# qqueing/DeepSpeaker-pytorch

Hardware: AMD Instinct MI355X
Metric: embeddings/sec (64-fbank x 160-frame utterances) (higher is better)
Workload: dtype f16

## Files before the change

deepspeaker-pytorch_amd/csrc/conv_block_f16.hip:

```cpp
#include <ds_device.h>
#include <algorithm>
#include <type_traits>
#include "ds_common.h"
#include "conv_mfma_f16_parts.h"

namespace {

constexpr int BK_R = 8;
constexpr int BK_CK = 32;
constexpr int BK_PS = 80;

struct BlockK {
    const _Float16 *x;
    const _Float16 *wa, *wb;
    const float *sa, *ha, *sb, *hb;
    void *y;
    int B, H, W, C;
    int tiles_per_img, n_tiles;
    int flags;
    unsigned y_bytes, x_bytes, y_plane_stride;
    const int *lens;
    int xcd_slots;
    unsigned *sched;
    int sched_lds;
#ifdef DS_F16_PROBE
    long long *probe;
#endif
};

#ifdef DS_F16_PROBE
#define DS_BLK_STAMP(i) do { if (p.probe && threadIdx.x == 0 && tile_no < 4) p.probe[((size_t)blockIdx.x * 4 + tile_no) * 8 + (i)] = (long long)__builtin_amdgcn_s_memtime(); } while (0)
#else
#define DS_BLK_STAMP(i) ((void)0)
#endif

#ifndef DS_BLOCK_RING
#define DS_BLOCK_RING 6
#endif

template <int WM, int WN, int NIT, bool MASKED = false>
__global__ void __launch_bounds__(WM * WN * 64) DS_ONE_WAVE_PER_SIMD conv_block3x3_f16_kernel(const BlockK p) {
    constexpr int NTHR = WM * WN * 64;
    constexpr int W = 16 * WM, WSH = WM == 2 ? 5 : 4;
    constexpr int MSA = 5, MSB = 4, NSUB = 2;
    constexpr int NT = 9, NU = 2 * NT, RU = DS_BLOCK_RING;
    constexpr int NMFA = MSA * NSUB, NMFB = MSB * NSUB;
    constexpr int SPU = (NMFA + 1) / 2 - NSUB;
    constexpr int UL = (NIT + SPU - 1) / SPU;
    constexpr int SPUB = NMFB / 2 - NSUB;
    constexpr int ROWS_A = BK_R + 2, ROWS_IN = BK_R + 4;
    using EG = ds_f16_epi<NSUB>;
    constexpr int TP = EG::TP, LPP = EG::LPP, PPI = EG::PPI, NRI = EG::NRI;
    constexpr int NRES = MSB * NRI, ULR = (NRES + SPUB - 1) / SPUB;
    static_assert(WM == 1 || WM == 2, "map width 16 or 32");
    static_assert(2 * UL <= NU && ULR + 2 <= NU && NU % RU == 0, "not enough units for the staging traffic");
    static_assert(NIT * NTHR == ROWS_IN * W * 4, "staging items must tile the input rows exactly");
    constexpr unsigned OOB = 0x80000000u;
    constexpr int pitch = W + 2;
    constexpr int tileA_bytes = ROWS_IN * pitch * BK_PS;

    char *lds = (char *)ds_dynamic_lds();
    const int tid = threadIdx.x, lane = tid & 63, wave = tid >> 6;
    const int wm = wave / WN, wn = wave % WN;
    const int l31 = lane & 31, lhi = lane >> 5;
    constexpr int C = WM == 2 ? 64 : 128;
    constexpr int RSB = C * 2 + 16;
    constexpr int n_chunks = C / BK_CK;
    const int n_base = wn * NSUB * 32;
    size_t lane_w = ds_f16_lane_w(n_base, l31, lhi);
    const size_t w_kc_stride = (size_t)NT * C * 16, w_tap_stride = (size_t)C * 16;
    auto w_unit = [&](const _Float16 *w, int chunk, int u) {
        return ds_f16_w_unit<NT, BK_CK / 16>(w, lane_w, w_kc_stride, w_tap_stride, chunk, u);
    };

    const int xcd = (int)blockIdx.x & 7, slot0 = (int)blockIdx.x >> 3;
    const int my_imgs = p.xcd_slots > 0 ? (p.B - xcd + 7) / 8 : 0;
    int t_cur = p.xcd_slots > 0 ? slot0 : (int)blockIdx.x;
    const int t_static = p.xcd_slots > 0 ? p.xcd_slots : (int)gridDim.x;
    const int t_end = p.xcd_slots > 0 ? my_imgs * p.tiles_per_img : p.n_tiles;
    unsigned *const q_next = p.sched + (p.xcd_slots > 0 ? xcd : 0);
    int *const sched_word = (int *)(lds + p.sched_lds);
    if (tid == 0) *sched_word = t_static + (int)ds_atomic_inc(q_next);
    __syncthreads();
    int t_next = ds_uniform(*sched_word);
    const float rcp_tpi = 1.0f / (float)p.tiles_per_img;
    auto tile_of = [&](int t, int &b, int &r0) {
        const int im = ds_div_small(t, p.tiles_per_img, rcp_tpi);
        r0 = (t - im * p.tiles_per_img) * BK_R;
        b = p.xcd_slots > 0 ? im * 8 + xcd : im;
    };

    unsigned g_rel[NIT];
    int l_off[NIT];
    {
        const int q = tid & 3, pix0 = tid >> 2;
#pragma unroll
        for (int it = 0; it < NIT; ++it) {
            const int pix = pix0 + it * (NTHR / 4);
            const int vr = pix >> WSH, c = pix & (W - 1);
            g_rel[it] = (unsigned)((pix * C + q * 8) * 2);
            l_off[it] = (vr * pitch + c + 1) * BK_PS + q * 16;
        }
    }
    const int lpix = ds_mfma_lpix(l31);
    int a_off[MSA];
#pragma unroll
    for (int ms = 0; ms < MSA; ++ms) {
        const int m = (wm * MSA + ms) * 32 + lpix;
        a_off[ms] = ((m >> WSH) * pitch + (m & (W - 1))) * BK_PS + 16 * lhi;
    }
    auto tap_off = [&](int tt, int rs) { return ((tt / 3) * pitch + (tt % 3)) * rs; };
    const ds_buffer ybuf = ds_make_buffer(p.y, p.y_bytes);
    const ds_buffer rbuf = ds_make_buffer(p.x, p.x_bytes);
    const int x_row_bytes = W * C * 2;
    const int my_c = (lane % LPP) * 8, my_p = lane / LPP;
    const int col = n_base + my_c;
    const bool out32 = (p.flags & DS_EPI_OUT_F32) != 0;
    float *tb = (float *)lds + wave * (2 * 32 * TP);

    auto stage_window = [&](int b, int r0, ds_buffer &xb, unsigned &lo) {
        const int h0 = r0 - 2;
        const int first = h0 < 0 ? -h0 : 0;
        const int last = p.H - h0 < ROWS_IN ? p.H - h0 : ROWS_IN;
        lo = (unsigned)(first * x_row_bytes);
        xb = ds_make_buffer((const char *)p.x + (size_t)(b * p.H + h0 + first) * x_row_bytes,
                            (unsigned)((last > first ? last - first : 0) * x_row_bytes));
    };

    f16x8 bq[RU][NSUB];
#pragma unroll
    for (int d = 0; d < RU; ++d)
#pragma unroll
        for (int ns = 0; ns < NSUB; ++ns) bq[d][ns] = *(const f16x8 *)(w_unit(p.wa, 0, d) + (size_t)ns * 32 * 16);

    f32x16 acc[MSA][NSUB];
    const f32x16 zero16 = {0.f, 0.f, 0.f, 0.f, 0.f, 0.f, 0.f, 0.f, 0.f, 0.f, 0.f, 0.f, 0.f, 0.f, 0.f, 0.f};

    f32x4 st[NIT];
    int b = 0, r0 = 0;
    ds_buffer xbuf = rbuf;
    unsigned x_lo = 0;
    if (t_cur < t_end) {
        tile_of(t_cur, b, r0);
        stage_window(b, r0, xbuf, x_lo);
#pragma unroll
        for (int it = 0; it < NIT; ++it) st[it] = ds_buffer_load_f32x4(xbuf, g_rel[it] - x_lo);
    }

    int tile_no = 0;
    (void)tile_no;
    for (; t_cur < t_end; ++tile_no) {
        DS_BLK_STAMP(0);
        int t_drawn = 0;
        if (tid == 0) t_drawn = t_static + (int)ds_atomic_inc(q_next);
        DS_OPAQUE_VGPR(lane_w);
        int h_valid = p.H;
        if (MASKED) {
            const int len = p.lens[b];
            h_valid = len < p.H ? len : p.H;
        }
        ds_lds_barrier();
        for (int i = tid; i < 2 * ROWS_IN * 2 * (BK_PS / 16); i += NTHR) {
            const int piece = i % (BK_PS / 16), rec = i / (BK_PS / 16);
            const int side = rec & 1, row = (rec >> 1) % ROWS_IN, buf = (rec >> 1) / ROWS_IN;
            *(f32x4 *)(lds + buf * tileA_bytes + (row * pitch + side * (W + 1)) * BK_PS + 16 * piece) = f32x4{0.0f, 0.0f, 0.0f, 0.0f};
        }
#pragma unroll
        for (int it = 0; it < NIT; ++it) *(f32x4 *)(lds + l_off[it]) = st[it];
        ds_lds_barrier();
        DS_BLK_STAMP(1);

        auto run_chunk = [&](auto first_tag, auto last_tag, int chunk, const char *buf, char *obuf) __attribute__((always_inline)) {
            constexpr bool FIRST = decltype(first_tag)::value, LAST = decltype(last_tag)::value;
            f16x8 a[2][MSA];
#pragma unroll
            for (int ms = 0; ms < MSA; ++ms) {
                DS_OPAQUE_VGPR(a_off[ms]);
                a[0][ms] = *(const f16x8 *)(buf + a_off[ms] + tap_off(0, BK_PS));
            }
            const unsigned xn = (unsigned)((chunk + 1) * BK_CK * 2) - x_lo;
            __builtin_amdgcn_sched_barrier(0);
#pragma unroll
            for (int u = 0; u < NU; ++u) {
                const int cur = u & 1, slot = u % RU;
                const bool more = u + 1 < NU;
                const char *nfrag = buf + tap_off((u + 1) % NT, BK_PS) + 32 * ((u + 1) / NT);
                const int ur = u - 1 + RU;
                const _Float16 *rw = (LAST && ur >= NU) ? w_unit(p.wb, 0, ur - NU)
                                                        : w_unit(p.wa, ur >= NU ? chunk + 1 : chunk, ur >= NU ? ur - NU : ur);
                const int rslot = (u + RU - 1) % RU;
#pragma unroll
                for (int q = 0; q < NMFA; ++q) {
                    const int ms = q / NSUB, ns = q % NSUB;
                    acc[ms][ns] = ds_mfma_32x32x16_f16(bq[slot][ns], a[cur][ms], (FIRST && u == 0) ? zero16 : acc[ms][ns]);
                    if (q & 1) {
                        const int lm = q >> 1;
#ifndef DS_ABL_NO_AFRAG
                        if (lm < MSA && more) a[cur ^ 1][lm] = *(const f16x8 *)(nfrag + a_off[lm]);
#endif
                    } else {
                        const int e = q >> 1;
                        if (e < NSUB) {
#ifndef DS_ABL_NO_REFILL
                            bq[rslot][e] = *(const f16x8 *)(rw + (size_t)e * 32 * 16);
#endif
                        } else if constexpr (!LAST) {
#ifndef DS_ABL_NO_STAGE
                            const int s = e - NSUB;
                            if (u < UL) {
                                const int it = u * SPU + s;
                                if (it < NIT) st[it] = ds_buffer_load_f32x4(xbuf, g_rel[it] + xn);
                            } else if (u >= NU - UL) {
                                const int it = (u - (NU - UL)) * SPU + s;
                                if (it < NIT) *(f32x4 *)(obuf + l_off[it]) = st[it];
                            }
#endif
                        }
                    }
                    __builtin_amdgcn_sched_barrier(0);
                }
            }
        };
        run_chunk(std::true_type{}, std::false_type{}, 0, lds, lds + tileA_bytes);
        ds_lds_barrier();
        for (int i = 1; i + 1 < n_chunks; ++i) {
            char *b0 = lds + (i & 1) * tileA_bytes, *b1 = lds + ((i & 1) ^ 1) * tileA_bytes;
            run_chunk(std::false_type{}, std::false_type{}, i, b0, b1);
            ds_lds_barrier();
        }
        run_chunk(std::false_type{}, std::true_type{}, n_chunks - 1, lds + ((n_chunks - 1) & 1) * tileA_bytes, lds);
        DS_BLK_STAMP(2);

        {
            f32x4 sca[NSUB][4], sha[NSUB][4];
#pragma unroll
            for (int ns = 0; ns < NSUB; ++ns)
#pragma unroll
                for (int g = 0; g < 4; ++g) {
                    const int c0 = n_base + ns * 32 + 8 * g + 4 * lhi;
                    sca[ns][g] = *(const f32x4 *)(p.sa + c0);
                    sha[ns][g] = *(const f32x4 *)(p.ha + c0);
                }
            ds_lds_barrier();
            const int ppr = RSB / 16;
            for (int i = tid; i < ROWS_A * 2 * ppr; i += NTHR) {
                const int piece = i % ppr, rec = i / ppr;
                *(f32x4 *)(lds + ((rec >> 1) * pitch + (rec & 1) * (W + 1)) * RSB + 16 * piece) = f32x4{0.0f, 0.0f, 0.0f, 0.0f};
            }
#pragma unroll
            for (int ms = 0; ms < MSA; ++ms) {
                const int m = (wm * MSA + ms) * 32 + lpix;
                const int i = m >> WSH, c = m & (W - 1);
                const int row = r0 - 1 + i;
                const unsigned keep = (row >= 0 && row < h_valid) ? 0xFFFFFFFFu : 0u;
                char *rec = lds + (i * pitch + c + 1) * RSB;
#pragma unroll
                for (int ns = 0; ns < NSUB; ++ns)
#pragma unroll
                    for (int g = 0; g < 4; ++g) {
                        ds_u32x2 hb;
#pragma unroll
                        for (int j2 = 0; j2 < 2; ++j2) {
                            const ds_f32x2 v = {acc[ms][ns][4 * g + 2 * j2], acc[ms][ns][4 * g + 2 * j2 + 1]};
                            const ds_f32x2 sc2 = {sca[ns][g][2 * j2], sca[ns][g][2 * j2 + 1]};
                            const ds_f32x2 sh2 = {sha[ns][g][2 * j2], sha[ns][g][2 * j2 + 1]};
                            ds_f32x2 t = v * sc2 + sh2;
                            t[0] = fminf(fmaxf(t[0], DS_F16_CLIP_LO), DS_F16_CLIP_HI);
                            t[1] = fminf(fmaxf(t[1], DS_F16_CLIP_LO), DS_F16_CLIP_HI);
                            hb[j2] = __builtin_bit_cast(unsigned, __builtin_convertvector(t, ds_f16x2)) & keep;
                        }
                        *(ds_u32x2 *)(rec + (n_base + ns * 32 + 8 * g + 4 * lhi) * 2) = hb;
                    }
            }
            ds_lds_barrier();
        }
        DS_BLK_STAMP(3);

        const int lin_base = (b * p.H + r0) * W;
        const int lin_valid = (p.H - r0 < BK_R ? p.H - r0 : BK_R) * W;
        f32x4 resv[MSB][NRI];
        {
            const int total = n_chunks * NU;
            int b_off[MSB];
#pragma unroll
            for (int ms = 0; ms < MSB; ++ms) {
                const int m = (wm * MSB + ms) * 32 + lpix;
                b_off[ms] = ((m >> WSH) * pitch + (m & (W - 1))) * RSB + 16 * lhi;
            }
            f16x8 a[2][MSB];
#pragma unroll
            for (int ms = 0; ms < MSB; ++ms) {
                DS_OPAQUE_VGPR(b_off[ms]);
                a[0][ms] = *(const f16x8 *)(lds + b_off[ms] + tap_off(0, RSB));
            }
            __builtin_amdgcn_sched_barrier(0);
            auto run_b = [&](auto first_tag, auto last_tag, int chunk) __attribute__((always_inline)) {
                constexpr bool FIRSTB = decltype(first_tag)::value, LASTB = decltype(last_tag)::value;
#pragma unroll
                for (int u = 0; u < NU; ++u) {
                    const int cur = u & 1, slot = u % RU;
                    const int gu = chunk * NU + u;
                    const bool more = gu + 1 < total;
                    const int nu = (u + 1) % NU, nchunk = (u + 1 < NU) ? chunk : chunk + 1;
                    const char *nfrag = lds + tap_off(nu % NT, RSB) + 32 * (nu / NT) + (more ? nchunk : chunk) * 64;
                    const int ur = u - 1 + RU;
                    const int rchunk = ur >= NU ? chunk + 1 : chunk;
                    const _Float16 *rw = rchunk < n_chunks ? w_unit(p.wb, rchunk, ur >= NU ? ur - NU : ur)
                                                           : w_unit(p.wa, 0, ur >= NU ? ur - NU : ur);
                    const int rslot = (u + RU - 1) % RU;
#pragma unroll
                    for (int q = 0; q < NMFB; ++q) {
                        const int ms = q / NSUB, ns = q % NSUB;
                        acc[ms][ns] = ds_mfma_32x32x16_f16(bq[slot][ns], a[cur][ms], (FIRSTB && u == 0) ? zero16 : acc[ms][ns]);
                        if (q & 1) {
                            const int lm = q >> 1;
#ifndef DS_ABL_NO_AFRAG
                            if (lm < MSB) a[cur ^ 1][lm] = *(const f16x8 *)(nfrag + b_off[lm]);
#endif
                        } else {
                            const int e = q >> 1;
                            if (e < NSUB) {
#ifndef DS_ABL_NO_REFILL
                                bq[rslot][e] = *(const f16x8 *)(rw + (size_t)e * 32 * 16);
#endif
                            } else if constexpr (LASTB) {
                                const int ri = (u - (NU - 2 - ULR)) * SPUB + (e - NSUB);
                                if (u >= NU - 2 - ULR && ri < NRES) {
                                    const int rms = ri / NRI, rk = ri % NRI;
                                    const int m = (wm * MSB + rms) * 32 + rk * PPI + my_p;
#ifdef DS_ABL_NO_RES
                                    resv[rms][rk] = f32x4{0.f, 0.f, 0.f, 0.f};
#else
                                    resv[rms][rk] = ds_buffer_load_f32x4(rbuf, m < lin_valid ? (unsigned)((lin_base + m) * C + col) * 2u
                                                                                            : DS_BUFFER_OOB);
#endif
                                }
                            }
                        }
                        __builtin_amdgcn_sched_barrier(0);
                    }
                }
            };
            run_b(std::true_type{}, std::false_type{}, 0);
            for (int chunk = 1; chunk + 1 < n_chunks; ++chunk) run_b(std::false_type{}, std::false_type{}, chunk);
            run_b(std::false_type{}, std::true_type{}, n_chunks - 1);
        }

        DS_BLK_STAMP(4);
        if (tid == 0) *sched_word = t_drawn;
        ds_lds_barrier();
        DS_BLK_STAMP(5);
        const int t_after = ds_uniform(*sched_word);
#ifndef DS_EPI_TABLES_LATE
        const f32x4 sc[2] = {*(const f32x4 *)(p.sb + col), *(const f32x4 *)(p.sb + col + 4)};
        const f32x4 sh[2] = {*(const f32x4 *)(p.hb + col), *(const f32x4 *)(p.hb + col + 4)};
        __builtin_amdgcn_sched_barrier(0);
#endif
        int nb = b, nr0 = r0;
        {
            const bool has_next = t_next < t_end;
            if (has_next) {
                tile_of(t_next, nb, nr0);
                stage_window(nb, nr0, xbuf, x_lo);
            } else {
                xbuf = ds_make_buffer(p.x, 0u);
                x_lo = 0;
            }
#pragma unroll
            for (int it = 0; it < NIT; ++it) st[it] = ds_buffer_load_f32x4(xbuf, g_rel[it] - x_lo);
        }
        const int lin_kept = (h_valid - r0) * W;
#ifdef DS_EPI_TABLES_LATE
        __builtin_amdgcn_sched_barrier(0);
        const f32x4 sc[2] = {*(const f32x4 *)(p.sb + col), *(const f32x4 *)(p.sb + col + 4)};
        const f32x4 sh[2] = {*(const f32x4 *)(p.hb + col), *(const f32x4 *)(p.hb + col + 4)};
#endif
        auto put_tile = [&](int ms) { ds_f16_put_tile<NSUB>(tb + (ms & 1) * (32 * TP), acc[ms], lpix, lhi); };
        const unsigned y_mul = p.y_plane_stride ? 16u : (unsigned)C;
        const unsigned y_add = p.y_plane_stride ? (unsigned)(col >> 4) * p.y_plane_stride + (unsigned)(col & 15) : (unsigned)col;
        auto write_out = [&](auto f32_tag) __attribute__((always_inline)) {
            constexpr bool OUT32 = decltype(f32_tag)::value;
            put_tile(0);
#pragma unroll
            for (int ms = 0; ms < MSB; ++ms) {
                const int cb = ms & 1;
                ds_wave_sync();
                const float *src = tb + cb * (32 * TP);
                f32x4 tv[NRI][2];
#pragma unroll
                for (int k = 0; k < NRI; ++k)
#pragma unroll
                    for (int hq = 0; hq < 2; ++hq) tv[k][hq] = *(const f32x4 *)(src + (k * PPI + my_p) * TP + my_c + 4 * hq);
                if (ms + 1 < MSB) put_tile(ms + 1);
#pragma unroll
                for (int k = 0; k < NRI; ++k) {
                    const f16x8 r8 = __builtin_bit_cast(f16x8, resv[ms][k]);
                    const int m = (wm * MSB + ms) * 32 + k * PPI + my_p;
                    const float keep = (!MASKED || m < lin_kept) ? DS_F16_CLIP_HI : DS_F16_CLIP_LO;
                    f32x4 o[2];
#pragma unroll
                    for (int hq = 0; hq < 2; ++hq)
#pragma unroll
                        for (int j2 = 0; j2 < 2; ++j2) {
                            const ds_f32x2 v = {tv[k][hq][2 * j2], tv[k][hq][2 * j2 + 1]};
                            const ds_f32x2 s2 = {sc[hq][2 * j2], sc[hq][2 * j2 + 1]}, h2 = {sh[hq][2 * j2], sh[hq][2 * j2 + 1]};
                            const ds_f16x2 rh = {r8[4 * hq + 2 * j2], r8[4 * hq + 2 * j2 + 1]};
                            ds_f32x2 t = v * s2 + h2;
                            t = t + __builtin_convertvector(rh, ds_f32x2);
                            o[hq][2 * j2] = fminf(fmaxf(t[0], DS_F16_CLIP_LO), keep);
                            o[hq][2 * j2 + 1] = fminf(fmaxf(t[1], DS_F16_CLIP_LO), keep);
                        }
                    const unsigned vo = m < lin_valid ? (unsigned)(lin_base + m) * y_mul + y_add : DS_BUFFER_OOB;
                    if constexpr (OUT32) {
                        const unsigned bo = vo != DS_BUFFER_OOB ? vo * 4u : DS_BUFFER_OOB;
                        ds_buffer_store_out_f32x4(ybuf, bo, o[0]);
                        ds_buffer_store_out_f32x4(ybuf, bo != DS_BUFFER_OOB ? bo + 16u : DS_BUFFER_OOB, o[1]);
                    } else {
                        ds_u32x4 hb;
#pragma unroll
                        for (int hq = 0; hq < 2; ++hq)
#pragma unroll
                            for (int j2 = 0; j2 < 2; ++j2)
                                hb[2 * hq + j2] = __builtin_bit_cast(unsigned, __builtin_convertvector(
                                                                                   ds_f32x2{o[hq][2 * j2], o[hq][2 * j2 + 1]}, ds_f16x2));
#ifdef DS_ABL_NO_STORE
                        if (hb[0] == 0x12345678u)
#endif
                        ds_buffer_store_out_f32x4(ybuf, vo != DS_BUFFER_OOB ? vo * 2u : DS_BUFFER_OOB, __builtin_bit_cast(f32x4, hb));
                    }
                }
            }
        };
        if (out32) write_out(std::true_type{});
        else write_out(std::false_type{});
        DS_BLK_STAMP(6);
        b = nb;
        r0 = nr0;
        t_cur = t_next;
        t_next = t_after;
    }
    if (tid == 0 && ds_atomic_inc(p.sched + DS_SCHED_DONE) == gridDim.x - 1) {
        for (int i = 0; i <= DS_SCHED_DONE; ++i) p.sched[i] = 0u;
    }
}

static size_t block_lds_bytes(int W, int C, int waves) {
    const size_t tileA = (size_t)(BK_R + 4) * (W + 2) * BK_PS;
    const size_t interm = (size_t)(BK_R + 2) * (W + 2) * (C * 2 + 16);
    const size_t epi = (size_t)2 * waves * 32 * ds_f16_epi<2>::TP * 4;
    return std::max(std::max(2 * tileA, interm), epi) + 64;
}

}

#ifdef DS_F16_PROBE
static long long *g_blk_probe = nullptr;
extern "C" void ds_block_set_probe(long long *buf) { g_blk_probe = buf; }
#endif


extern "C" int ds_conv_block_f16_supported(int B, int H, int W, int C) {
    if (B <= 0 || H <= 0) return 0;
    if ((long long)B * H * W * C >= (1ll << 30)) return 0;
    return (W == 32 && C == 64) || (W == 16 && C == 128);
}

static int conv_block_f16(const void *x_f16, const void *wa_f16, const void *wb_f16, const float *scale_a,
                          const float *shift_a, const float *scale_b, const float *shift_b, void *y, const int *lens,
                          int B, int H, int W, int C, int flags, void *stream) {
    DS_REQUIRE(x_f16 && wa_f16 && wb_f16 && scale_a && shift_a && scale_b && shift_b && y, DS_ERR_NULL);
    DS_REQUIRE(ds_conv_block_f16_supported(B, H, W, C), DS_ERR_UNSUPPORTED);
    DS_REQUIRE(DS_ALIGNED16(x_f16) && DS_ALIGNED16(wa_f16) && DS_ALIGNED16(wb_f16) && DS_ALIGNED16(y) &&
                   DS_ALIGNED16(scale_a) && DS_ALIGNED16(shift_a) && DS_ALIGNED16(scale_b) && DS_ALIGNED16(shift_b),
               DS_ERR_ALIGNMENT);
    DS_REQUIRE(!((flags & DS_EPI_OUT_F32) && (flags & DS_EPI_OUT_PLANES16)), DS_ERR_UNSUPPORTED);
    BlockK k;
    k.x = (const _Float16 *)x_f16; k.wa = (const _Float16 *)wa_f16; k.wb = (const _Float16 *)wb_f16;
    k.sa = scale_a; k.ha = shift_a; k.sb = scale_b; k.hb = shift_b; k.y = y;
    k.B = B; k.H = H; k.W = W; k.C = C;
    k.tiles_per_img = ds_ceil_div(H, BK_R);
    k.n_tiles = B * k.tiles_per_img;
    k.flags = flags;
    const long long n = (long long)B * H * W * C;
    k.x_bytes = (unsigned)(n * 2);
    k.y_bytes = (unsigned)(n * ((flags & DS_EPI_OUT_F32) ? 4 : 2));
    k.y_plane_stride = (flags & DS_EPI_OUT_PLANES16) ? (unsigned)((long long)B * H * W * 16) : 0u;
    k.lens = lens;
#ifdef DS_F16_PROBE
    k.probe = g_blk_probe;
#endif
    const int resident = 2 * ds_cu_count();
    int grid = k.n_tiles < resident ? k.n_tiles : resident;
    k.xcd_slots = 0;
    if (B >= 8 && grid == resident && resident % 8 == 0) k.xcd_slots = resident / 8;
    k.sched = ds_sched_slot(stream);
    DS_REQUIRE(k.sched != nullptr, DS_ERR_NO_WORKSPACE);
    k.sched_lds = (int)block_lds_bytes(W, C, 2) - 16;
    if (C == 64) {
        if (lens) DS_LAUNCH_BIG_LDS((conv_block3x3_f16_kernel<2, 1, 12, true>), grid, 128, block_lds_bytes(W, C, 2), stream, k);
        else DS_LAUNCH_BIG_LDS((conv_block3x3_f16_kernel<2, 1, 12>), grid, 128, block_lds_bytes(W, C, 2), stream, k);
    } else {
        if (lens) DS_LAUNCH_BIG_LDS((conv_block3x3_f16_kernel<1, 2, 6, true>), grid, 128, block_lds_bytes(W, C, 2), stream, k);
        else DS_LAUNCH_BIG_LDS((conv_block3x3_f16_kernel<1, 2, 6>), grid, 128, block_lds_bytes(W, C, 2), stream, k);
    }
    return ds_last_launch_error();
}

extern "C" int ds_conv_block_f16(const void *x_f16, const void *wa_f16, const void *wb_f16, const float *scale_a,
                                 const float *shift_a, const float *scale_b, const float *shift_b, void *y, int B, int H,
                                 int W, int C, int flags, void *stream) {
    return conv_block_f16(x_f16, wa_f16, wb_f16, scale_a, shift_a, scale_b, shift_b, y, nullptr, B, H, W, C, flags, stream);
}

extern "C" int ds_conv_block_f16_masked(const void *x_f16, const void *wa_f16, const void *wb_f16, const float *scale_a,
                                        const float *shift_a, const float *scale_b, const float *shift_b, void *y,
                                        const int *lens, int B, int H, int W, int C, int flags, void *stream) {
    DS_REQUIRE(lens != nullptr, DS_ERR_NULL);
    return conv_block_f16(x_f16, wa_f16, wb_f16, scale_a, shift_a, scale_b, shift_b, y, lens, B, H, W, C, flags, stream);
}
```

Baseline: 397,000.

## Cache BN tables in LDS, template output type, rework tile scheduling draw

Copies the four batch-norm scale/shift vectors into LDS once per block and reads epilogue tables from there instead of global memory. Makes the f32 output mode a template parameter so the epilogue branch is resolved at compile time. Replaces the float-reciprocal tile division with a host-computed magic multiplier, moves the atomic tile draw to after the compute and publishes it through LDS, and adds dummy out-of-bounds stores plus opaque-register and schedule barriers and extra probe stamps. The changes raise LDS use per block and add new sync ordering for the scheduler word.

```diff
diff --git a/deepspeaker-pytorch_amd/csrc/conv_block_f16.hip b/deepspeaker-pytorch_amd/csrc/conv_block_f16.hip
--- a/deepspeaker-pytorch_amd/csrc/conv_block_f16.hip
+++ b/deepspeaker-pytorch_amd/csrc/conv_block_f16.hip
@@ -17,6 +17,7 @@
     void *y;
     int B, H, W, C;
     int tiles_per_img, n_tiles;
+    unsigned tpi_magic;
     int flags;
     unsigned y_bytes, x_bytes, y_plane_stride;
     const int *lens;
@@ -29,16 +30,26 @@
 };
 
 #ifdef DS_F16_PROBE
-#define DS_BLK_STAMP(i) do { if (p.probe && threadIdx.x == 0 && tile_no < 4) p.probe[((size_t)blockIdx.x * 4 + tile_no) * 8 + (i)] = (long long)__builtin_amdgcn_s_memtime(); } while (0)
+#define DS_BLK_STAMP(i) do { if (p.probe && threadIdx.x == 0 && tile_no < 4) p.probe[((size_t)blockIdx.x * 4 + tile_no) * 24 + (i)] = (long long)__builtin_amdgcn_s_memtime(); } while (0)
+#define DS_BLK_STAMP_IN(i) do { __builtin_amdgcn_sched_barrier(0); DS_BLK_STAMP(i); __builtin_amdgcn_sched_barrier(0); } while (0)
 #else
 #define DS_BLK_STAMP(i) ((void)0)
+#define DS_BLK_STAMP_IN(i) ((void)0)
 #endif
 
 #ifndef DS_BLOCK_RING
 #define DS_BLOCK_RING 6
 #endif
 
-template <int WM, int WN, int NIT, bool MASKED = false>
+__device__ __forceinline__ unsigned blk_draw(unsigned *q) {
+#if defined(__HIP_DEVICE_COMPILE__)
+    return __builtin_amdgcn_atomic_inc32(q, 0xFFFFFFFFu, __ATOMIC_RELAXED, "agent");
+#else
+    return ds_atomic_inc(q);
+#endif
+}
+
+template <int WM, int WN, int NIT, bool MASKED = false, bool OUT32 = false>
 __global__ void __launch_bounds__(WM * WN * 64) DS_ONE_WAVE_PER_SIMD conv_block3x3_f16_kernel(const BlockK p) {
     constexpr int NTHR = WM * WN * 64;
     constexpr int W = 16 * WM, WSH = WM == 2 ? 5 : 4;
@@ -81,11 +92,18 @@
     unsigned *const q_next = p.sched + (p.xcd_slots > 0 ? xcd : 0);
     int *const sched_word = (int *)(lds + p.sched_lds);
     if (tid == 0) *sched_word = t_static + (int)ds_atomic_inc(q_next);
+    float *const bn_tab = (float *)(lds + p.sched_lds + 16);
+    for (int i = tid; i < C; i += NTHR) {
+        bn_tab[i] = p.sa[i];
+        bn_tab[C + i] = p.ha[i];
+        bn_tab[2 * C + i] = p.sb[i];
+        bn_tab[3 * C + i] = p.hb[i];
+    }
     __syncthreads();
     int t_next = ds_uniform(*sched_word);
-    const float rcp_tpi = 1.0f / (float)p.tiles_per_img;
     auto tile_of = [&](int t, int &b, int &r0) {
-        const int im = ds_div_small(t, p.tiles_per_img, rcp_tpi);
+        int im = (int)(((unsigned long long)(unsigned)t * p.tpi_magic) >> 32);
+        im += ((im + 1) * p.tiles_per_img <= t) ? 1 : 0;
         r0 = (t - im * p.tiles_per_img) * BK_R;
         b = p.xcd_slots > 0 ? im * 8 + xcd : im;
     };
@@ -115,7 +133,6 @@
     const int x_row_bytes = W * C * 2;
     const int my_c = (lane % LPP) * 8, my_p = lane / LPP;
     const int col = n_base + my_c;
-    const bool out32 = (p.flags & DS_EPI_OUT_F32) != 0;
     float *tb = (float *)lds + wave * (2 * 32 * TP);
 
     auto stage_window = [&](int b, int r0, ds_buffer &xb, unsigned &lo) {
@@ -145,14 +162,15 @@
         stage_window(b, r0, xbuf, x_lo);
 #pragma unroll
         for (int it = 0; it < NIT; ++it) st[it] = ds_buffer_load_f32x4(xbuf, g_rel[it] - x_lo);
+#pragma unroll
+        for (int i = 0; i < NRES * (OUT32 ? 2 : 1); ++i)
+            ds_buffer_store_out_f32x4(ybuf, DS_BUFFER_OOB - 16u * (unsigned)i, f32x4{0.0f, 0.0f, 0.0f, 0.0f});
     }
 
     int tile_no = 0;
     (void)tile_no;
     for (; t_cur < t_end; ++tile_no) {
         DS_BLK_STAMP(0);
-        int t_drawn = 0;
-        if (tid == 0) t_drawn = t_static + (int)ds_atomic_inc(q_next);
         DS_OPAQUE_VGPR(lane_w);
         int h_valid = p.H;
         if (MASKED) {
@@ -160,6 +178,7 @@
             h_valid = len < p.H ? len : p.H;
         }
         ds_lds_barrier();
+        t_next = ds_uniform(*sched_word);
         for (int i = tid; i < 2 * ROWS_IN * 2 * (BK_PS / 16); i += NTHR) {
             const int piece = i % (BK_PS / 16), rec = i / (BK_PS / 16);
             const int side = rec & 1, row = (rec >> 1) % ROWS_IN, buf = (rec >> 1) / ROWS_IN;
@@ -238,8 +257,8 @@
 #pragma unroll
                 for (int g = 0; g < 4; ++g) {
                     const int c0 = n_base + ns * 32 + 8 * g + 4 * lhi;
-                    sca[ns][g] = *(const f32x4 *)(p.sa + c0);
-                    sha[ns][g] = *(const f32x4 *)(p.ha + c0);
+                    sca[ns][g] = *(const f32x4 *)(bn_tab + c0);
+                    sha[ns][g] = *(const f32x4 *)(bn_tab + C + c0);
                 }
             ds_lds_barrier();
             const int ppr = RSB / 16;
@@ -247,6 +266,7 @@
                 const int piece = i % ppr, rec = i / ppr;
                 *(f32x4 *)(lds + ((rec >> 1) * pitch + (rec & 1) * (W + 1)) * RSB + 16 * piece) = f32x4{0.0f, 0.0f, 0.0f, 0.0f};
             }
+            DS_BLK_STAMP_IN(12);
 #pragma unroll
             for (int ms = 0; ms < MSA; ++ms) {
                 const int m = (wm * MSA + ms) * 32 + lpix;
@@ -271,6 +291,7 @@
                         }
                         *(ds_u32x2 *)(rec + (n_base + ns * 32 + 8 * g + 4 * lhi) * 2) = hb;
                     }
+                DS_BLK_STAMP_IN(13 + ms);
             }
             ds_lds_barrier();
         }
@@ -347,15 +368,12 @@
         }
 
         DS_BLK_STAMP(4);
-        if (tid == 0) *sched_word = t_drawn;
+        unsigned drawn = 0;
+        if (tid == 0) drawn = blk_draw(q_next);
         ds_lds_barrier();
         DS_BLK_STAMP(5);
-        const int t_after = ds_uniform(*sched_word);
-#ifndef DS_EPI_TABLES_LATE
-        const f32x4 sc[2] = {*(const f32x4 *)(p.sb + col), *(const f32x4 *)(p.sb + col + 4)};
-        const f32x4 sh[2] = {*(const f32x4 *)(p.hb + col), *(const f32x4 *)(p.hb + col + 4)};
-        __builtin_amdgcn_sched_barrier(0);
-#endif
+        const f32x4 sc[2] = {*(const f32x4 *)(bn_tab + 2 * C + col), *(const f32x4 *)(bn_tab + 2 * C + col + 4)};
+        const f32x4 sh[2] = {*(const f32x4 *)(bn_tab + 3 * C + col), *(const f32x4 *)(bn_tab + 3 * C + col + 4)};
         int nb = b, nr0 = r0;
         {
             const bool has_next = t_next < t_end;
@@ -370,20 +388,18 @@
             for (int it = 0; it < NIT; ++it) st[it] = ds_buffer_load_f32x4(xbuf, g_rel[it] - x_lo);
         }
         const int lin_kept = (h_valid - r0) * W;
-#ifdef DS_EPI_TABLES_LATE
-        __builtin_amdgcn_sched_barrier(0);
-        const f32x4 sc[2] = {*(const f32x4 *)(p.sb + col), *(const f32x4 *)(p.sb + col + 4)};
-        const f32x4 sh[2] = {*(const f32x4 *)(p.hb + col), *(const f32x4 *)(p.hb + col + 4)};
-#endif
         auto put_tile = [&](int ms) { ds_f16_put_tile<NSUB>(tb + (ms & 1) * (32 * TP), acc[ms], lpix, lhi); };
         const unsigned y_mul = p.y_plane_stride ? 16u : (unsigned)C;
         const unsigned y_add = p.y_plane_stride ? (unsigned)(col >> 4) * p.y_plane_stride + (unsigned)(col & 15) : (unsigned)col;
-        auto write_out = [&](auto f32_tag) __attribute__((always_inline)) {
-            constexpr bool OUT32 = decltype(f32_tag)::value;
+        auto write_out = [&]() __attribute__((always_inline)) {
+            DS_BLK_STAMP_IN(7);
             put_tile(0);
 #pragma unroll
             for (int ms = 0; ms < MSB; ++ms) {
                 const int cb = ms & 1;
+                __builtin_amdgcn_sched_barrier(0);
+#pragma unroll
+                for (int k = 0; k < NRI; ++k) DS_OPAQUE_VGPR(resv[ms][k]);
                 ds_wave_sync();
                 const float *src = tb + cb * (32 * TP);
                 f32x4 tv[NRI][2];
@@ -429,27 +445,28 @@
                         ds_buffer_store_out_f32x4(ybuf, vo != DS_BUFFER_OOB ? vo * 2u : DS_BUFFER_OOB, __builtin_bit_cast(f32x4, hb));
                     }
                 }
+                DS_BLK_STAMP_IN(8 + ms);
             }
         };
-        if (out32) write_out(std::true_type{});
-        else write_out(std::false_type{});
+        write_out();
         DS_BLK_STAMP(6);
         b = nb;
         r0 = nr0;
+        if (tid == 0) *sched_word = t_static + (int)drawn;
         t_cur = t_next;
-        t_next = t_after;
     }
     if (tid == 0 && ds_atomic_inc(p.sched + DS_SCHED_DONE) == gridDim.x - 1) {
         for (int i = 0; i <= DS_SCHED_DONE; ++i) p.sched[i] = 0u;
     }
 }
 
-static size_t block_lds_bytes(int W, int C, int waves) {
+static size_t block_sched_lds(int W, int C, int waves) {
     const size_t tileA = (size_t)(BK_R + 4) * (W + 2) * BK_PS;
     const size_t interm = (size_t)(BK_R + 2) * (W + 2) * (C * 2 + 16);
     const size_t epi = (size_t)2 * waves * 32 * ds_f16_epi<2>::TP * 4;
-    return std::max(std::max(2 * tileA, interm), epi) + 64;
-}
+    return std::max(std::max(2 * tileA, interm), epi) + 64 - 16;
+}
+static size_t block_lds_bytes(int W, int C, int waves) { return block_sched_lds(W, C, waves) + 16 + (size_t)4 * C * sizeof(float); }
 
 }
 
@@ -480,6 +497,7 @@
     k.B = B; k.H = H; k.W = W; k.C = C;
     k.tiles_per_img = ds_ceil_div(H, BK_R);
     k.n_tiles = B * k.tiles_per_img;
+    k.tpi_magic = k.tiles_per_img == 1 ? 0xFFFFFFFFu : (unsigned)((1ull << 32) / (unsigned)k.tiles_per_img);
     k.flags = flags;
     const long long n = (long long)B * H * W * C;
     k.x_bytes = (unsigned)(n * 2);
@@ -495,14 +513,19 @@
     if (B >= 8 && grid == resident && resident % 8 == 0) k.xcd_slots = resident / 8;
     k.sched = ds_sched_slot(stream);
     DS_REQUIRE(k.sched != nullptr, DS_ERR_NO_WORKSPACE);
-    k.sched_lds = (int)block_lds_bytes(W, C, 2) - 16;
-    if (C == 64) {
-        if (lens) DS_LAUNCH_BIG_LDS((conv_block3x3_f16_kernel<2, 1, 12, true>), grid, 128, block_lds_bytes(W, C, 2), stream, k);
-        else DS_LAUNCH_BIG_LDS((conv_block3x3_f16_kernel<2, 1, 12>), grid, 128, block_lds_bytes(W, C, 2), stream, k);
-    } else {
-        if (lens) DS_LAUNCH_BIG_LDS((conv_block3x3_f16_kernel<1, 2, 6, true>), grid, 128, block_lds_bytes(W, C, 2), stream, k);
-        else DS_LAUNCH_BIG_LDS((conv_block3x3_f16_kernel<1, 2, 6>), grid, 128, block_lds_bytes(W, C, 2), stream, k);
-    }
+    k.sched_lds = (int)block_sched_lds(W, C, 2);
+    const size_t lds_bytes = block_lds_bytes(W, C, 2);
+    const bool out32 = (flags & DS_EPI_OUT_F32) != 0;
+#define DS_BLOCK_LAUNCH(WM, WN, NIT)                                                                                              \
+    do {                                                                                                                          \
+        if (lens && out32) DS_LAUNCH_BIG_LDS((conv_block3x3_f16_kernel<WM, WN, NIT, true, true>), grid, 128, lds_bytes, stream, k);   \
+        else if (lens) DS_LAUNCH_BIG_LDS((conv_block3x3_f16_kernel<WM, WN, NIT, true, false>), grid, 128, lds_bytes, stream, k);      \
+        else if (out32) DS_LAUNCH_BIG_LDS((conv_block3x3_f16_kernel<WM, WN, NIT, false, true>), grid, 128, lds_bytes, stream, k);     \
+        else DS_LAUNCH_BIG_LDS((conv_block3x3_f16_kernel<WM, WN, NIT, false, false>), grid, 128, lds_bytes, stream, k);               \
+    } while (0)
+    if (C == 64) DS_BLOCK_LAUNCH(2, 1, 12);
+    else DS_BLOCK_LAUNCH(1, 2, 6);
+#undef DS_BLOCK_LAUNCH
     return ds_last_launch_error();
 }
 
```

Result: no change. 400,500 (median of 6 runs) (+0.9%).
